# worldbench/lidarcrafter

Measured on AMD Instinct MI355X. Metric: denoising-steps/sec, nuScenes 32×1024 range image, 1/2/4/8 GPU, higher is better.
Workload: dtype f16x2-split MFMA, fp32 accumulate (fp32-class accuracy)

## Files before the change

### lidarcrafter_amd/csrc/conv_f16x2.hip

```cpp
#include "conv_f16x2_common.h"

using namespace lcconv;

namespace {

#if LC_TIMING
__device__ unsigned long long lc_dbg[32];
#endif

#ifndef LC_NP_AUX
#define LC_NP_AUX LC_DEF_AUX
#endif
template <class C, bool WIDE = false, bool EMIT = false>
__global__ __launch_bounds__(256, (C::BN > 64 && C::NTAP == 9) ? 1 : 2) void conv_f16x2_kernel(ConvArgsH a) {
    constexpr int HALO = C::HALO, NTAP = C::NTAP, BN = C::BN;
    constexpr int XR = C::XR, XW = C::XW;
    constexpr int KS = 2 * HALO + 1;
    constexpr int CB = (NTAP == 1 && WIDE) ? ((BN <= 64 && C::TH_ * C::TW_ <= 128) ? 8 : 4) : C::CB;
    constexpr int XU = CB * XR * XW, NXU = (XU + 255) / 256;
    constexpr int WU = NTAP * CB * BN, NWU = (WU + 255) / 256;
    __shared__ half8 lds[2 * XU + 2 * WU];
    __shared__ f32x4 ctab[GN_MAX_C];
    __shared__ float2 gtab[GN_MAX_G];
    half8* xh = lds;
// ... 641 lines not shown
        while (t < 4 && extent % (t * 2) == 0 && n_tiles / (t * 2) >= 256) t *= 2;
        return t;
    };
    static const int vert_env = [] { const char* e = getenv("LC_CONV_VERT"); return e ? atoi(e) : 1; }();
    static const int xcd_env = [] { const char* e = getenv("LC_CONV_XCD"); return e ? atoi(e) : 1; }();
    const int tpb_h = max_tpb(a.tiles_h), tpb_w = max_tpb(a.tiles_w);
    int vert = vert_env && tpb_h >= tpb_w;
    int tpb = vert ? tpb_h : tpb_w;
    if (C::NTAP == 1) tpb = 1;
    if (a.tpb > 0) {
        tpb = a.tpb;
        vert = vert_env && a.tiles_h % tpb == 0;
        if (!vert && a.tiles_w % tpb) tpb = 1;
    }
    if (a.part) tpb = 1;
    a.tpb = tpb;
    a.vert = vert;
    dim3 grid(a.B * a.tiles_h * a.tiles_w / tpb, ncot);
    a.xcd = (xcd_env && grid.x % 8 == 0 && grid.x >= 16) ? 1 : 0;

    if (a.xsp) {
        if constexpr (C::NTAP == 9) {
            if (a.part) grid.z = a.ksplit;
            if (a.ostats && !a.part) hipLaunchKernelGGL((conv_f16x2_ps_kernel<C, true>), grid, dim3(C::NT), 0, st, a);
            else hipLaunchKernelGGL((conv_f16x2_ps_kernel<C, false>), grid, dim3(C::NT), 0, st, a);
            return lc_launch_status();
        } else {
            return LC_EUNSUP;
        }
    }
    {
        const long long d = (const char*)a.wl - (const char*)a.wh;
        if (d <= 0 || d >= (1ll << 31)) return LC_EINVAL;
        if (d + (long long)C::NTAP * a.Cib * a.Cop * 16 >= (1ll << 31)) return LC_EUNSUP;
    }
    const int gnm = a.gn ? (a.gn_silu ? 1 : 2) : 0;
#define LC_PIPE_LAUNCH(E, G) hipLaunchKernelGGL((conv_f16x2_pipe_kernel<C, E, G>), grid, dim3(C::NT), 0, st, a)
    if (a.ostats && a.ounit == 2) {
        if constexpr (C::NTAP == 9) {
            if (gnm == 1) LC_PIPE_LAUNCH(2, 1); else if (gnm == 2) LC_PIPE_LAUNCH(2, 2); else LC_PIPE_LAUNCH(2, 0);
        } else {
            return LC_EUNSUP;
        }
    } else if (a.ostats) {
        if (gnm == 1) LC_PIPE_LAUNCH(1, 1); else if (gnm == 2) LC_PIPE_LAUNCH(1, 2); else LC_PIPE_LAUNCH(1, 0);
    } else {
// ... 333 lines not shown
extern "C" int lc_range_from_amax(const float* amax, int64_t n, float bound_mult, lc_conv_range* range, lc_stream_t s) {
    if (!amax || n <= 0 || !range || !(bound_mult >= 1.0f)) return LC_EINVAL;
    hipLaunchKernelGGL(range_from_amax_kernel, dim3(1), dim3(256), 0, lc_s(s), range, amax, (long long)n, bound_mult);
    return lc_launch_status();
}

extern "C" int lc_conv2d_ring_f16x2_fwd(const float* x, int64_t x_bs, const void* wp_hi,
                                        const void* wp_lo, const float* bias, const float* res,
                                        int64_t res_bs, float* y, int64_t y_bs, int B, int Ci,
                                        int Co, int H, int W, int ks, float out_scale, int tile_cfg,
                                        const float* gn_coeffs, int gn_cpad, int gn_silu,
                                        const lc_gn_stats_input* gn_stats, float* gn_ostats_out, int gn_ostats_unit,
                                        const float* wmeta, lc_conv_range* range, lc_stream_t s) {
    if (!x || !wp_hi || !wp_lo || !y || !wmeta || !range || B <= 0 || Ci <= 0 || Co <= 0 || H <= 0 ||
        W <= 0)
        return LC_EINVAL;
    if (ks != 1 && ks != 3) return LC_EUNSUP;
    if ((long long)H * W >= (1 << 24)) return LC_EUNSUP;
    if ((long long)Ci * H * W * 4 >= (1ll << 31) || (long long)Co * H * W * 4 >= (1ll << 31)) return LC_EUNSUP;
    ConvArgsH a;
    a.x = x; a.wh = (const half8*)wp_hi; a.wl = (const half8*)wp_lo; a.bias = bias; a.res = res;
    a.y = y; a.x_bs = x_bs; a.res_bs = res_bs; a.y_bs = y_bs;
    a.range = range; a.wmeta = wmeta;
    a.xsp = nullptr; a.xsp_bs = 0; a.xsp_c8 = 0; a.part = nullptr; a.ksplit = 0;
    a.B = B; a.Ci = Ci; a.Co = Co; a.H = H; a.W = W;
    a.Cib = (Ci + 15) / 16 * 2; a.Cop = (Co + 63) / 64 * 64;
    a.out_scale = out_scale;
    a.tiles_h = a.tiles_w = 0;
    a.gn = reinterpret_cast<const f32x4*>(gn_coeffs);
    a.Cgn = gn_cpad; a.gn_silu = gn_silu;
    a.gs = lc_gn_stats_input{nullptr, 0, 0, 0.f, nullptr, nullptr, nullptr, nullptr, 0, nullptr, nullptr};
    a.segs = STAT_SEGS_NONE;
    if (gn_stats) {
        if (gn_coeffs || gn_stats->G <= 0 || Ci % gn_stats->G) return LC_EINVAL;
        if (gn_stats->partials) {
            if (gn_stats->nch <= 0) return LC_EINVAL;
        } else {
            if (const int rc = stat_segs_from(gn_stats->os0, gn_stats->os1, Ci, Ci / gn_stats->G, LC_EINVAL, a.segs)) return rc;
            if (gn_stats->G > GN_MAX_G) return LC_EUNSUP;
        }
        a.gs = *gn_stats;
        a.gs.os0 = a.gs.os1 = nullptr;
        a.gn = reinterpret_cast<const f32x4*>(x);
        a.Cgn = gn_cpad > 0 ? gn_cpad : (Ci + 15) / 16 * 16;
    }
    a.tpb = 0;
    if (tile_cfg >= 100) { a.tpb = tile_cfg / 100; tile_cfg %= 100; }
// ... 40 lines not shown
                                           lc_conv_range* range, lc_stream_t s) {
    if (!x_split || !wp_hi || !wp_lo || (!y && !splitk_part) || !wmeta || !range || B <= 0 || Ci <= 0 ||
        Co <= 0 || H <= 0 || W <= 0)
        return LC_EINVAL;
    if (Ci % 16) return LC_EUNSUP;
    if (splitk_part && (ksplit < 2 || ksplit > Ci / 16)) return LC_EINVAL;
    if ((long long)H * W >= (1 << 24) || (long long)2 * (Ci / 8) * H * W * 16 >= (1ll << 31)) return LC_EUNSUP;
    if ((long long)Co * H * W * 4 >= (1ll << 31)) return LC_EUNSUP;
    ConvArgsH a;
    a.x = nullptr; a.wh = (const half8*)wp_hi; a.wl = (const half8*)wp_lo; a.bias = bias; a.res = res;
    a.y = y; a.x_bs = 0; a.res_bs = res_bs; a.y_bs = y_bs;
    a.range = range; a.wmeta = wmeta;
    a.B = B; a.Ci = Ci; a.Co = Co; a.H = H; a.W = W;
    a.Cib = Ci / 8; a.Cop = (Co + 63) / 64 * 64;
    if (a.wl != a.wh + (long long)9 * a.Cib * a.Cop) return LC_EINVAL;
    a.xsp = (const half8*)x_split; a.xsp_c8 = Ci / 8; a.xsp_bs = (long long)2 * (Ci / 8) * H * W;
    a.part = splitk_part; a.ksplit = splitk_part ? ksplit : 0;
    a.out_scale = out_scale;
    a.tiles_h = a.tiles_w = 0;
    a.gn = nullptr; a.Cgn = 0; a.gn_silu = 0;
    a.gs = lc_gn_stats_input{nullptr, 0, 0, 0.f, nullptr, nullptr, nullptr, nullptr, 0, nullptr, nullptr};
    a.segs = STAT_SEGS_NONE;
    a.tpb = 0;
    if (tile_cfg >= 100) { a.tpb = tile_cfg / 100; tile_cfg %= 100; }
    if (tile_cfg == 0) tile_cfg = auto_cfg_h(B, Ci < 24 ? 24 : Ci, Co, H, W, 3);
    if (pipe_stat_slots(tile_cfg, H, W) <= 0) return LC_EUNSUP;
    a.ostats = nullptr; a.oslots = 0; a.ounit = 8;
    if (gn_ostats_out && !splitk_part) {
        a.oslots = pipe_stat_slots(tile_cfg, H, W);
        if (Co % 8 || (gn_ostats_unit != 8 && gn_ostats_unit != 4)) return LC_EUNSUP;
        a.ostats = reinterpret_cast<f32x4*>(gn_ostats_out);
        a.ounit = gn_ostats_unit;
    }
    return dispatch_h<3>(tile_cfg, a, lc_s(s));
}

#include "conv_f16x2_ps1.h"

namespace {
__global__ __launch_bounds__(256) void splitk_reduce_kernel(const float* __restrict__ part, int ks,
                                                           const float* __restrict__ bias,
                                                           const float* __restrict__ res,
                                                           long long res_bs, float* __restrict__ y,
                                                           long long y_bs, int B, int Co, int HW,
                                                           float out_scale, f32x4* __restrict__ ostats,
                                                           int oslots) {
// ... 70 lines not shown
```

### lidarcrafter_amd/csrc/conv_f16x2_common.h

```cpp
#pragma once
#include <cstdlib>
#include <type_traits>

#include "common.h"
#include "f16x2.h"
#include "stats_entry.h"

#ifndef LC_EPI_MODE
#define LC_EPI_MODE 2
#endif

namespace lcconv {


__device__ __forceinline__ void epi_store(float* p, float v) {
#if LC_EPI_MODE == 2
    asm volatile("global_store_dword %0, %1, off sc1" :: "v"(p), "v"(v) : "memory");
#elif LC_EPI_MODE == 3
    asm volatile("global_store_dword %0, %1, off nt" :: "v"(p), "v"(v) : "memory");
#else
    *p = v;
#endif
}

// ... 34 lines not shown
    const float* bias;
    const float* res;
    float* y;
    lc_conv_range* range;
    const float* wmeta;
    const half8* xsp;
    long long xsp_bs;
    int xsp_c8;
    float* part;
    int ksplit;
    long long x_bs, res_bs, y_bs;
    int B, Ci, Co, H, W, Cib, Cop;
    int tiles_h, tiles_w;
    float out_scale;
    const f32x4* gn;
    int Cgn, gn_silu;
    lc_gn_stats_input gs;
    StatSegs segs;
    int tpb;
    int vert;
    int xcd;
    f32x4* ostats;
    int oslots, ounit;
};

constexpr int GN_MAX_C = 1024;

__device__ __forceinline__ f32x4 gn_row_from_stats(const lc_gn_stats_input& gs, const float* xb,
                                                   int b, int c, int C, long long HW) {
    f32x4 r = {0.f, 0.f, 0.f, 0.f};
    if (c >= C) return r;
    const int cpg = C / gs.G, g = c / cpg;
    const double* pp = gs.partials + ((long long)b * gs.G + g) * gs.nch * 2;
    double s_ = 0.0, q_ = 0.0;
    typedef double f64x2 __attribute__((ext_vector_type(2)));
    const f64x2* pv = reinterpret_cast<const f64x2*>(pp);
    for (int k0 = 0; k0 < gs.nch; k0 += 8) {
        f64x2 v[8];
#pragma unroll
        for (int k = 0; k < 8; ++k) v[k] = k0 + k < gs.nch ? pv[k0 + k] : f64x2{0.0, 0.0};
#pragma unroll
        for (int k = 0; k < 8; ++k)
            if (k0 + k < gs.nch) { s_ += v[k].x; q_ += v[k].y; }
    }
    const double n = (double)cpg * (double)HW;
    const double dm = s_ / n;
// ... 288 lines not shown
```

### lidarcrafter_amd/csrc/conv_f16x2_ps.h

```cpp
#pragma once

template <class C, bool EMIT_STATS, bool S2 = false>
__global__ __launch_bounds__(C::NT, C::NT / 256) void conv_f16x2_ps_kernel(ConvArgsH a) {
    constexpr int CB = C::CB, HALO = C::HALO, NTAP = C::NTAP, BN = C::BN;
    constexpr int XR = S2 ? 3 * C::TH_ : C::XR, XW = S2 ? 2 * C::TW_ + 1 : C::XW, XU = CB * XR * XW, WU = C::WU;
    static_assert(!S2 || (C::TH_ == 1 && NTAP == 9), "stride-2 form: 3x3, one output row per tile");
    constexpr int KS = 2 * HALO + 1;
    constexpr int NT = C::NT, NWV = NT / 64;
    constexpr int NXI = (XU + 63) / 64, NWI = (WU + 63) / 64;
    constexpr int XS = NXI * 64, WS = NWI * 64;
    constexpr int KX = (2 * NXI + NWV - 1) / NWV, KW = (2 * NWI + NWV - 1) / NWV;
    constexpr int IPW = KX + KW;
#ifndef LC_PS_SPT
#define LC_PS_SPT 0
#endif
    constexpr int SPT = LC_PS_SPT ? LC_PS_SPT : (IPW + NTAP - 1) / NTAP;
    constexpr int BUF = 2 * XS + 2 * WS + 64;
    constexpr unsigned OOB = 0x80000000u;
    __shared__ half8 lds[2 * BUF];
    const int tid = threadIdx.x;
    const int lane = tid & 63;
    const int wave = __builtin_amdgcn_readfirstlane(tid >> 6);
    const int wco = wave / C::WPX_, wpx = wave % C::WPX_;

    const int tpb = a.tpb;
    int bx = blockIdx.x;
    if (a.xcd) bx = (bx & 7) * (gridDim.x >> 3) + (bx >> 3);
    int tw_i, th_i;
    if (a.vert) {
// ... 22 lines not shown
    __amdgpu_buffer_rsrc_t rs_w = __builtin_amdgcn_make_buffer_rsrc((void*)a.wh, 0, 2u * wplane * 16u,
                                                                    0x00020000);

    unsigned voff[IPW];
    int ldsoff[IPW];
#pragma unroll
    for (int k = 0; k < IPW; ++k) {
        if (k < KX) {
            const int j = wave + k * NWV;
            const int plane = j / NXI;
            ldsoff[k] = j < 2 * NXI ? plane * XS + (j - plane * NXI) * 64 : 2 * XS + 2 * WS;
        } else {
            const int j = wave + (k - KX) * NWV;
            const int plane = j / NWI;
            ldsoff[k] = j < 2 * NWI ? 2 * XS + plane * WS + (j - plane * NWI) * 64 : 2 * XS + 2 * WS;
        }
    }
    auto set_offsets = [&](int h0t, int w0t, bool weights_too) {
#pragma unroll
        for (int k = 0; k < IPW; ++k) {
            if (k < KX) {
                const int j = wave + k * NWV;
                const int plane = j / NXI, e = (j - plane * NXI) * 64 + lane;
                const int cb = e / (XR * XW), rem = e - cb * (XR * XW);
                const int r = rem / XW, c = rem - r * XW;
                if constexpr (S2) {
                    const int ky = r;
                    int row = 2 * h0t + ky;
                    if (h0t == 0 && ky == 2) row = 2 * H + 1;
                    if (h0t == H - 1 && ky == 0) row = 2 * H + 2;
                    int col;
                    if (c <= C::TW_) { col = w0t + c; col = col >= W ? col - W : col; }
                    else col = W + w0t + (c - C::TW_ - 1);
                    const bool ok = j < 2 * NXI && e < XU && h0t < H;
                    voff[k] = ok ? (unsigned)(((plane * C8 + cb) * XROWS + row) * XCOLS + col) * 16u : OOB;
                    continue;
                }
                const int gh = h0t - HALO + r;
                int gw = w0t - HALO + c;
                gw %= W; if (gw < 0) gw += W;
                const bool ok = j < 2 * NXI && e < XU && gh >= 0 && gh < H;
                voff[k] = ok ? (unsigned)(((plane * C8 + cb) * H + gh) * W + gw) * 16u : OOB;
            } else if (weights_too) {
                const int j = wave + (k - KX) * NWV;
                const int plane = j / NWI, e = (j - plane * NWI) * 64 + lane;
                const int row = e / BN, cu = e - row * BN;
                const int tap = row / CB, cb = row - tap * CB;
                voff[k] = (j < 2 * NWI && e < WU)
                              ? ((unsigned)((tap * a.Cib + cb) * a.Cop + co0 + cu) + plane * wplane) * 16u
                              : OOB;
            }
        }
    };
    set_offsets(h0, w0, true);
    const unsigned x_chunk = (unsigned)CB * (unsigned)(XROWS * XCOLS) * 16u;
    const unsigned w_chunk = (unsigned)CB * (unsigned)a.Cop * 16u;
    auto issue_slot = [&](half8* buf, int k, unsigned xso, unsigned wso) {
        if (LC_PS_ABL & 1) return;
        if (k < KX) {
            if (!(LC_PS_ABL & 4)) lds_dma16(rs_x, (lds_vptr)(buf + ldsoff[k]), voff[k], xso);
        } else {
            if (!(LC_PS_ABL & 8)) lds_dma16(rs_w, (lds_vptr)(buf + ldsoff[k]), voff[k], wso);
        }
    };
    auto issue = [&](half8* buf, int ch) {
#pragma unroll
        for (int k = 0; k < IPW; ++k) issue_slot(buf, k, (unsigned)ch * x_chunk, (unsigned)ch * w_chunk);
    };

    f32x16 acc[C::TCO_][C::TPX_];
#pragma unroll
    for (int i = 0; i < C::TCO_; ++i)
#pragma unroll
        for (int j = 0; j < C::TPX_; ++j)
#pragma unroll
            for (int r = 0; r < 16; ++r) acc[i][j][r] = 0.0f;

    const int kh = lane >> 5, l31 = lane & 31;
    int xbase[C::TPX_];
#pragma unroll
    for (int j = 0; j < C::TPX_; ++j) {
        const int t = wpx * C::TPX_ + j;
        const int tr = t / C::TPR, tc = t - tr * C::TPR;
        xbase[j] = kh * (XR * XW) + (S2 ? 3 * tr : tr) * XW + tc * 32 + l31;
    }
    const int wbase = kh * BN + wco * C::TCO_ * 32 + l31;

    auto compute = [&](const half8* cur, half8* nxt, int nxt_ch) {
        const unsigned xso = (unsigned)nxt_ch * x_chunk, wso = (unsigned)nxt_ch * w_chunk;
        const half8* cxh = cur;
        const half8* cxl = cur + XS;
        const half8* cwh = cur + 2 * XS;
        const half8* cwl = cwh + WS;
        half8 ah[2][C::TCO_], al[2][C::TCO_], bh[2][C::TPX_], bl[2][C::TPX_];
        auto fetch = [&](int tap, int s) {
            const int dy = tap / KS, dx = tap - dy * KS;
#pragma unroll
            for (int i = 0; i < C::TCO_; ++i) {
                ah[s][i] = cwh[tap * CB * BN + wbase + i * 32];
                al[s][i] = cwl[tap * CB * BN + wbase + i * 32];
            }
#pragma unroll
            for (int j = 0; j < C::TPX_; ++j) {
                const int o = S2 ? dy * XW + (dx == 1 ? C::TW_ + 1 : (dx == 2 ? 1 : 0)) : dy * XW + dx;
                bh[s][j] = cxh[xbase[j] + o];
                bl[s][j] = cxl[xbase[j] + o];
            }
        };
        fetch(0, 0);
// ... 14 lines not shown
                        acc[i][j] = __builtin_amdgcn_mfma_f32_32x32x16_f16(al[s][i], bh[s][j], acc[i][j], 0, 0, 0);
            }
            if (LC_F16X2_TERMS & 4) {
#pragma unroll
                for (int i = 0; i < C::TCO_; ++i)
#pragma unroll
                    for (int j = 0; j < C::TPX_; ++j)
                        acc[i][j] = __builtin_amdgcn_mfma_f32_32x32x16_f16(ah[s][i], bl[s][j], acc[i][j], 0, 0, 0);
            }
#pragma unroll
            for (int i = 0; i < C::TCO_; ++i)
#pragma unroll
                for (int j = 0; j < C::TPX_; ++j)
                    acc[i][j] = __builtin_amdgcn_mfma_f32_32x32x16_f16(ah[s][i], bh[s][j], acc[i][j], 0, 0, 0);
            if (LC_PS_SCHED == 1) {
#pragma unroll
                for (int q = 0; q < 3 * C::TCO_ * C::TPX_; ++q) {
                    __builtin_amdgcn_sched_group_barrier(0x008, 1, 0);
                    __builtin_amdgcn_sched_group_barrier(0x100, 1, 0);
                }
            }
        }
        __builtin_amdgcn_sched_barrier(0);
    };

    half8* cur = lds;
    half8* nxt = lds + BUF;
    const int nchunk = a.Cib / CB;
    const int ksp = a.part ? a.ksplit : 1;
    const int ch_lo = (int)blockIdx.z * nchunk / ksp, ch_hi = ((int)blockIdx.z + 1) * nchunk / ksp;
    const int last = ch_hi - 1;
    issue(cur, ch_lo);
    const int co_wave = co0 + wco * C::TCO_ * 32 + 4 * kh;
    float bias_r[C::TCO_][16];
#pragma unroll
    for (int i = 0; i < C::TCO_; ++i)
#pragma unroll
        for (int r = 0; r < 16; ++r) {
            const int co = co_wave + i * 32 + mfma_row(r);
            bias_r[i][r] = (a.bias && co < a.Co) ? a.bias[co] : 0.0f;
        }
    float res_r[C::TCO_][C::TPX_][16];
    const float* rb = a.res ? a.res + (long long)b * a.res_bs : nullptr;
    const unsigned HW4 = (unsigned)HW * 4u;
    const __amdgpu_buffer_rsrc_t rs_yb = __builtin_amdgcn_make_buffer_rsrc(
        (void*)(a.y + (long long)b * a.y_bs), 0, (unsigned)a.Co * HW4, 0x00020000);
// ... 3 lines not shown
        const int t = wpx * C::TPX_ + j;
        const int tr = t / C::TPR, tc = t - tr * C::TPR;
        const int gh = h0 + tr, gw = w0 + tc * 32 + l31;
        return (gh < H && gw < W) ? (unsigned)(co_wave * HW + gh * W + gw) * 4u : OOB;
    };
    auto prefetch_res = [&]() {
#pragma unroll
        for (int j = 0; j < C::TPX_; ++j) {
            const unsigned vo = px_off(j);
#pragma unroll
            for (int i = 0; i < C::TCO_; ++i)
#pragma unroll
                for (int r = 0; r < 16; ++r) {
                    const int cor = i * 32 + mfma_row(r);
                    res_r[i][j][r] = (LC_PS_ABL & 16) ? 0.0f : __builtin_bit_cast(float, __builtin_amdgcn_raw_buffer_load_b32(
                        rs_rb, co_wave + cor < a.Co ? vo : OOB, (unsigned)cor * HW4, 0));
                }
        }
    };
    asm volatile("s_waitcnt vmcnt(0)" ::: "memory");
    __syncthreads();
    auto k_iter = [&](int nxt_ch) {
        if (LC_PS_ABL & 2) issue(nxt, nxt_ch);
        else compute(cur, nxt, nxt_ch);
        asm volatile("s_waitcnt vmcnt(0)" ::: "memory");
        __syncthreads();
        half8* t = cur; cur = nxt; nxt = t;
    };
    for (int tile = 0; tile < tpb; ++tile) {
        for (int ch = ch_lo; ch < last; ++ch) k_iter(ch + 1);
        if (!a.part) prefetch_res();
        const bool more = tile + 1 < tpb;
        if (more) set_offsets(h0 + dh, w0 + dw, false);
        k_iter(more ? ch_lo : last);
        if (a.part) {
            float* pb = a.part + ((long long)blockIdx.z * a.B + b) * a.Co * HW;
#pragma unroll
            for (int j = 0; j < C::TPX_; ++j) {
                const int t = wpx * C::TPX_ + j;
                const int tr = t / C::TPR, tc = t - tr * C::TPR;
                const int gh = h0 + tr, gw = w0 + tc * 32 + l31;
                const bool pok = gh < H && gw < W;
                const long long poff = (long long)gh * W + gw;
#pragma unroll
                for (int i = 0; i < C::TCO_; ++i)
#pragma unroll
                    for (int r = 0; r < 16; ++r) {
                        const int co = co_wave + i * 32 + mfma_row(r);
                        if (pok && co < a.Co) epi_store(&pb[(long long)co * HW + poff], acc[i][j][r] * out_unscale);
                        acc[i][j][r] = 0.0f;
                    }
            }
            h0 += dh; w0 += dw;
            continue;
        }
        StatAcc<PIVOT_HALF_RT> st[C::TCO_][4];
        const bool quads = a.ounit == 4, upper_quad = quads && (lane & 32);
// ... 50 lines not shown
```

### lidarcrafter_amd/csrc/conv_f16x2_s2.hip

```cpp
#include "conv_f16x2_common.h"

using namespace lcconv;

namespace {

#include "conv_f16x2_ps.h"

__global__ __launch_bounds__(256) void fir_down2_prefilter_split_kernel(
    const float* __restrict__ x, long long x_bs, half8* __restrict__ ysp, int C8, int H, int W, int nstrip, int strip_len,
    lc_conv_range* range) {
    const int Wh = W >> 1;
    const int i = blockIdx.x * 256 + threadIdx.x;
    const int c8 = blockIdx.y;
    const int b = blockIdx.z / nstrip, strip = blockIdx.z - b * nstrip;
    const float xs = range->x_scale, seen = range->amax_scaled;
    float am = 0.f;
    if (i < Wh) {
        const long long HW = (long long)H * W;
        const float* xb = x + b * x_bs + (long long)c8 * 8 * HW;
        const int R = H + 3;
        half8* yh = ysp + ((long long)b * 2 * C8 + c8) * R * W;
        half8* yl = yh + (long long)C8 * R * W;
        const int cm1 = (2 * i - 1 + W) % W, cp2 = (2 * i + 2) % W;
        constexpr float f0 = 0.125f, f1 = 0.375f, f2 = 0.375f, f3 = 0.125f;
// ... 306 lines not shown
    dim3 grid((W / 2 + 255) / 256, C / 8, B * nstrip);
    hipLaunchKernelGGL(fir_down2_prefilter_split_kernel, grid, dim3(256), 0, lc_s(s), x, (long long)x_bs,
                       reinterpret_cast<half8*>(y_split), C / 8, H, W, nstrip, strip_len, range);
    return lc_launch_status();
}

extern "C" int lc_conv2d_ring_s2_f16x2_ps_fwd(const void* x_split, const void* wp_hi, const void* wp_lo, const float* bias,
                                              float* y, int64_t y_bs, int B, int Ci, int Co, int Ho, int Wo, float out_scale,
                                              float* gn_ostats_out, int gn_ostats_unit, const float* wmeta,
                                              lc_conv_range* range, lc_stream_t s) {
    using C = S2Cfg;
    if (!x_split || !wp_hi || !wp_lo || !y || !wmeta || !range || B <= 0 || Ci <= 0 || Co <= 0 || Ho <= 0 || Wo <= 0)
        return LC_EINVAL;
    if (Ci % 16 || Ho < 2 || Wo % C::TW_) return LC_EUNSUP;
    const long long plane_units = (long long)(Ci / 8) * (2 * Ho + 3) * (2 * Wo);
    if (2 * plane_units * 16 >= (1ll << 31) || (long long)Co * Ho * Wo * 4 >= (1ll << 31)) return LC_EUNSUP;
    ConvArgsH a;
    a.x = nullptr; a.wh = (const half8*)wp_hi; a.wl = (const half8*)wp_lo; a.bias = bias; a.res = nullptr;
    a.y = y; a.x_bs = 0; a.res_bs = 0; a.y_bs = y_bs;
    a.range = range; a.wmeta = wmeta;
    a.B = B; a.Ci = Ci; a.Co = Co; a.H = Ho; a.W = Wo;
    a.Cib = Ci / 8; a.Cop = (Co + 63) / 64 * 64;
    if (a.wl != a.wh + (long long)9 * a.Cib * a.Cop) return LC_EINVAL;
    a.xsp = (const half8*)x_split; a.xsp_c8 = Ci / 8; a.xsp_bs = 2 * plane_units;
    a.part = nullptr; a.ksplit = 0;
    a.out_scale = out_scale;
    a.gn = nullptr; a.Cgn = 0; a.gn_silu = 0;
    a.gs = lc_gn_stats_input{nullptr, 0, 0, 0.f, nullptr, nullptr, nullptr, nullptr, 0, nullptr, nullptr};
    a.segs = STAT_SEGS_NONE;
    a.ostats = nullptr; a.oslots = 0; a.ounit = 8;
    if (gn_ostats_out) {
        if (Co % 8 || (gn_ostats_unit != 8 && gn_ostats_unit != 4)) return LC_EUNSUP;
        a.oslots = (int)lc_conv2d_ring_s2_stats_slots(Ho, Wo);
        a.ostats = reinterpret_cast<f32x4*>(gn_ostats_out);
        a.ounit = gn_ostats_unit;
    }
    a.tiles_h = Ho; a.tiles_w = Wo / C::TW_;
    const int ncot = (Co + C::BN - 1) / C::BN;
    const long long n_tiles = (long long)B * a.tiles_h * a.tiles_w * ncot;
    int tpb = 1;
    while (tpb < 4 && a.tiles_h % (tpb * 2) == 0 && n_tiles / (tpb * 2) >= 256) tpb *= 2;
    a.tpb = tpb; a.vert = 1;
    dim3 grid(B * a.tiles_h * a.tiles_w / tpb, ncot);
    a.xcd = (grid.x % 8 == 0 && grid.x >= 16) ? 1 : 0;
    static const int form_env = [] { const char* e = getenv("LC_S2_FORM"); return e ? atoi(e) : 2; }();
    if (form_env == 1) {
        if (a.ostats) hipLaunchKernelGGL((conv_f16x2_ps_kernel<C, true, true>), grid, dim3(C::NT), 0, lc_s(s), a);
// ... 17 lines not shown
```

### lidarcrafter_amd/ops.py

```python
from __future__ import annotations

from typing import Optional

import torch

from ._lib import check, lib

_F32 = torch.float32
_HALF = (torch.float16, torch.bfloat16)


def _stream() -> int:
    return torch.cuda.current_stream().cuda_stream


def _req(t: torch.Tensor, name: str) -> None:
    if not isinstance(t, torch.Tensor) or not t.is_cuda:
        raise RuntimeError(f"lidarcrafter_amd.ops: `{name}` must be a CUDA(HIP) tensor -- the hot "
                           "path has no CPU fallback (oracle/ holds the CPU restatement for tests)")
    if t.dtype != _F32:
        raise TypeError(f"`{name}` must be float32, got {t.dtype} (float16 / bfloat16 INPUTS are "
                        "up-cast at the op boundary, e.g. under torch.autocast; `out=` tensors and "
                        "other dtypes are not)")

# ... 815 lines not shown
            sbuf, slots = None, 0
            unit = 2 if (emit_stats is not True and int(emit_stats) in (2, 4)) else 8
            if emit_stats and PRODUCER_GN_STATS and (unit == 8 or ks == 3):
                slots = int(lib().lc_conv2d_ring_f16x2_stats_slots(B, Ci, Co, H, W, ks, int(tile_cfg)))
                if slots > 0:
                    sbuf = torch.empty((B, Co // unit, slots, 4), device=x.device, dtype=_F32)
            check(_conv_lib().lc_conv2d_ring_f16x2_fwd(x.data_ptr(), x_bs, wh.data_ptr(), wl.data_ptr(),
                                                 _p(bias), _p(res), r_bs, out.data_ptr(), y_bs, B,
                                                 Ci, Co, H, W, ks, float(out_scale),
                                                 int(tile_cfg), _p(gn_coeffs), cpad, int(gn_silu),
                                                 gs_ref, _p(sbuf), unit, packed.wmeta.data_ptr(),
                                                 packed.range_ptr(x.device), _stream()),
                  "lc_conv2d_ring_f16x2_fwd")
            if sbuf is not None:
                _attach_stats(out, _OctStatsHandle(sbuf, Co, slots, (B, H * W), unit))
        else:
            check(lib().lc_conv2d_ring_fwd(x.data_ptr(), x_bs, wp.data_ptr(), _p(bias), _p(res),
                                           r_bs, out.data_ptr(), y_bs, B, Ci, Co, H, W, ks,
                                           float(out_scale), int(tile_cfg), _stream()),
                  "lc_conv2d_ring_fwd")
    return out


def _conv2d_ring_presplit(xs: SplitAct, packed: PackedConv, weight, bias, res, out, out_scale,
                          tile_cfg, emit_stats) -> torch.Tensor:
    if xs.packed is not packed:
        raise ValueError("conv: the pre-split activation was produced for another layer "
                         "(its x_scale belongs to that layer's range record)")
    wh, wl = packed.get_f16x2(weight)
    B, Ci, H, W = xs.shape
    if Ci != packed.Ci or packed.ks not in (1, 3):
        raise ValueError("conv: pre-split input needs a 1x1 / 3x3 kernel with matching channels")
    Co = packed.Co
    dev = xs.buf.device
    if out is None:
        out = torch.empty((B, Co, H, W), device=dev, dtype=_F32)
    y_bs = _bs4(out, "out")
    if tuple(out.shape) != (B, Co, H, W):
        raise ValueError(f"conv: out shape {tuple(out.shape)} != {(B, Co, H, W)}")
    r_bs = 0
    if res is not None:
        r_bs = _bs4(res, "res")
        if tuple(res.shape) != (B, Co, H, W):
            raise ValueError("conv: residual shape mismatch")
    if bias is not None:
        _req(bias, "bias")
    _drop_stats(out)
    if packed.ks == 1:
        with _Timed("conv1x1", 2.0 * B * H * W * Co * Ci):
            check(_conv_lib().lc_conv1x1_f16x2_ps_fwd(xs.buf.data_ptr(), wh.data_ptr(), wl.data_ptr(), _p(bias), _p(res),
                                                      r_bs, out.data_ptr(), y_bs, B, Ci, Co, H, W, float(out_scale),
                                                      packed.wmeta.data_ptr(), packed.range_ptr(dev), _stream()),
                  "lc_conv1x1_f16x2_ps_fwd")
        return out
    ks = splitk_factor(B, Ci, Co, H, W) if tile_cfg == 0 else 0
    sk_cfg = 0
    if _SPLITK_FORCE and tile_cfg == 0 and Ci >= _SPLITK_FORCE[2]:
        ks, sk_cfg = _SPLITK_FORCE[0], _SPLITK_FORCE[1]
    with _Timed("conv3x3", 2.0 * B * H * W * Co * Ci * 9,
                rd=4.0 * (B * Ci * H * W + Co * Ci * 9 + (B * Co * H * W if res is not None else 0)),
                wr=4.0 * B * Co * H * W):
        sbuf, slots = None, 0
        unit = 8 if emit_stats is True else int(emit_stats or 0)
        want_stats = unit in (8, 4) and PRODUCER_GN_STATS and Co % 8 == 0
        if ks >= 2:
            part = torch.empty((ks, B, Co, H, W), device=dev, dtype=_F32)
            check(_conv_lib().lc_conv2d_ring_f16x2_ps_fwd(xs.buf.data_ptr(), wh.data_ptr(), wl.data_ptr(),
                                                    None, None, 0, None, 0, B, Ci, Co, H, W, 1.0, sk_cfg,
                                                    None, 8, part.data_ptr(), ks,
                                                    packed.wmeta.data_ptr(), packed.range_ptr(dev),
                                                    _stream()), "lc_conv2d_ring_f16x2_ps_fwd")
            if want_stats and unit == 8:
                slots = int(lib().lc_splitk_stats_slots(H, W))
                sbuf = torch.empty((B, Co // 8, slots, 4), device=dev, dtype=_F32)
            check(lib().lc_splitk_reduce(part.data_ptr(), ks, _p(bias), _p(res), r_bs, out.data_ptr(),
                                         y_bs, B, Co, H, W, float(out_scale), _p(sbuf), _stream()),
                  "lc_splitk_reduce")
        else:
            if want_stats:
                slots = int(lib().lc_conv2d_ring_f16x2_stats_slots(B, max(Ci, 24), Co, H, W, 3,
                                                                   int(tile_cfg)))
                if slots > 0:
                    sbuf = torch.empty((B, Co // unit, slots, 4), device=dev, dtype=_F32)
            check(_conv_lib().lc_conv2d_ring_f16x2_ps_fwd(xs.buf.data_ptr(), wh.data_ptr(), wl.data_ptr(),
                                                    _p(bias), _p(res), r_bs, out.data_ptr(), y_bs, B,
                                                    Ci, Co, H, W, float(out_scale), int(tile_cfg),
                                                    _p(sbuf), unit if sbuf is not None else 8, None, 0,
                                                    packed.wmeta.data_ptr(),
                                                    packed.range_ptr(dev), _stream()),
                  "lc_conv2d_ring_f16x2_ps_fwd")
        if sbuf is not None:
            _attach_stats(out, _OctStatsHandle(sbuf, Co, slots, (B, H * W), unit))
    return out


FOLD_DOWN = _os.environ.get("LC_FOLD_DOWN", "1") != "0"


def can_fold_down(Ci: int, Co: int, H: int, W: int) -> bool:
    return (FOLD_DOWN and PRESPLIT and CONV_PRECISION == "f16x2" and conv_products() == 3 and Ci % 16 == 0 and
            Co % 8 == 0 and H % 2 == 0 and H >= 4 and W % 128 == 0)


def conv_down2(x: torch.Tensor, packed: PackedConv, weight, bias, out: Optional[torch.Tensor] = None,
               emit_stats=False) -> torch.Tensor:
    x_bs = _bs4(x, "x")
    B, Ci, H, W = x.shape
    wh, wl = packed.get_f16x2(weight)
    Co = packed.Co
# ... 1553 lines not shown
```

Baseline: 285.8.

## Add 16x16x32 MFMA body for presplit 3x3 conv with three-product f16x2

Adds an alternative compute path to the presplit 3x3 convolution kernel that uses 16x16x32 MFMA instructions instead of 32x32x16. It pairs taps across the K dimension so the nine taps fit into five steps, pads the per-channel-block LDS image to a multiple of 16, and converts the 16x16 accumulators back into the 32x32 layout with permlane16 swaps before the epilogue. The path is on by default through an env flag, and a tile_cfg offset of 1000 can disable it. A microbenchmark comparing the two MFMA shapes is also added. The trade-off is slightly more MFMA slots per chunk, one zero-padded tap, and extra register pressure from the second accumulator set.

```diff
diff --git a/devtools/ubench/mfma_shape.hip b/devtools/ubench/mfma_shape.hip
--- /dev/null
+++ b/devtools/ubench/mfma_shape.hip
@@ -0,0 +1,185 @@
+#include <hip/hip_runtime.h>
+#include <stdio.h>
+#include <stdlib.h>
+#include <algorithm>
+#include <vector>
+typedef _Float16 half8 __attribute__((ext_vector_type(8)));
+typedef float f32x16 __attribute__((ext_vector_type(16)));
+typedef float f32x4 __attribute__((ext_vector_type(4)));
+
+constexpr int CBS = 400;
+constexpr int XW = 66;
+constexpr int XS = 832, WS = 1152;
+constexpr int IMG = 2 * XS + 2 * WS;
+
+__device__ __forceinline__ void fill(half8* lds, const half8* in) {
+    for (int e = threadIdx.x; e < IMG; e += blockDim.x) lds[e] = in[e];
+    __syncthreads();
+}
+
+struct Stamp { unsigned long long c0, c1, r0, r1; };
+__device__ __forceinline__ void stamp0(Stamp& s) { s.c0 = __builtin_amdgcn_s_memtime(); s.r0 = __builtin_amdgcn_s_memrealtime(); }
+__device__ __forceinline__ void stamp1(Stamp& s, unsigned long long* st) {
+    s.c1 = __builtin_amdgcn_s_memtime(); s.r1 = __builtin_amdgcn_s_memrealtime();
+    if (threadIdx.x == 0) { st[2 * blockIdx.x] = s.c1 - s.c0; st[2 * blockIdx.x + 1] = s.r1 - s.r0; }
+}
+
+__global__ __launch_bounds__(512, 2) void k32(float* out, const half8* in, unsigned long long* st, int chunks) {
+    __shared__ half8 lds[IMG];
+    fill(lds, in);
+    const int lane = threadIdx.x & 63, wave = threadIdx.x >> 6;
+    const int kh = lane >> 5, l31 = lane & 31;
+    const half8 *cxh = lds, *cxl = lds + XS, *cwh = lds + 2 * XS, *cwl = cwh + WS;
+    const int wco = wave >> 2, wpx = wave & 3;
+    const int xb = kh * CBS + wpx * XW + l31, wb = kh * 64 + wco * 32 + l31;
+    f32x16 acc[2];
+    for (int j = 0; j < 2; ++j) for (int r = 0; r < 16; ++r) acc[j][r] = 0.f;
+    Stamp s; stamp0(s);
+    for (int ch = 0; ch < chunks; ++ch) {
+        asm volatile("" ::: "memory");
+        half8 ah[2], al[2], bh[2][2], bl[2][2];
+        auto fetch = [&](int tap, int q) {
+            const int o = (tap / 3) * XW + tap % 3;
+            ah[q] = cwh[tap * 128 + wb]; al[q] = cwl[tap * 128 + wb];
+            for (int j = 0; j < 2; ++j) { bh[q][j] = cxh[xb + o + 32 * j]; bl[q][j] = cxl[xb + o + 32 * j]; }
+        };
+        fetch(0, 0);
+#pragma unroll
+        for (int tap = 0; tap < 9; ++tap) {
+            const int q = tap & 1;
+            __builtin_amdgcn_sched_barrier(0);
+            if (tap + 1 < 9) fetch(tap + 1, q ^ 1);
+            __builtin_amdgcn_sched_barrier(0);
+#pragma unroll
+            for (int j = 0; j < 2; ++j) acc[j] = __builtin_amdgcn_mfma_f32_32x32x16_f16(al[q], bh[q][j], acc[j], 0, 0, 0);
+#pragma unroll
+            for (int j = 0; j < 2; ++j) acc[j] = __builtin_amdgcn_mfma_f32_32x32x16_f16(ah[q], bl[q][j], acc[j], 0, 0, 0);
+#pragma unroll
+            for (int j = 0; j < 2; ++j) acc[j] = __builtin_amdgcn_mfma_f32_32x32x16_f16(ah[q], bh[q][j], acc[j], 0, 0, 0);
+        }
+        __builtin_amdgcn_sched_barrier(0);
+        __syncthreads();
+    }
+    stamp1(s, st);
+    float t = 0;
+    for (int j = 0; j < 2; ++j) for (int r = 0; r < 16; ++r) t += acc[j][r];
+    out[blockIdx.x * blockDim.x + threadIdx.x] = t;
+}
+
+__global__ __launch_bounds__(512, 2) void k16(float* out, const half8* in, unsigned long long* st, int chunks) {
+    __shared__ half8 lds[IMG];
+    fill(lds, in);
+    const int lane = threadIdx.x & 63, wave = threadIdx.x >> 6;
+    const int g = lane >> 4, p = lane & 15, cb = g & 1, t2 = g >> 1;
+    const int pi = (p & 3) | ((p & 4) << 1) | ((p & 8) >> 1);
+    const int wco = wave >> 2, wpx = wave & 3;
+    const int xrow = cb * CBS + wpx * XW + p, wrow = cb * 64 + wco * 32 + pi;
+    const int xb1 = xrow + t2, xb2 = xrow + t2 * XW, xb8 = xrow + t2 * XS;
+    const int wb1 = wrow + t2 * 128, wb2 = wrow + t2 * 384, wb8 = wrow + (1 - t2) * WS;
+    const half8 *cxh = lds, *cxl = lds + XS, *cwh = lds + 2 * XS, *cwl = cwh + WS;
+    f32x4 acc[2][4];
+    for (int a = 0; a < 2; ++a) for (int j = 0; j < 4; ++j) for (int r = 0; r < 4; ++r) acc[a][j][r] = 0.f;
+    Stamp s; stamp0(s);
+    for (int ch = 0; ch < chunks; ++ch) {
+        asm volatile("" ::: "memory");
+        half8 ah[2][2], al[2][2], bh[2][4], bl[2][4];
+        auto fetch = [&](int step, int q, int part) {
+            if (step < 4) {
+                const int t0 = step == 3 ? 2 : 3 * step;
+                const int o = (t0 / 3) * XW + t0 % 3, xb = step == 3 ? xb2 : xb1, wb = step == 3 ? wb2 : wb1;
+                if (part == 0) {
+                    for (int a = 0; a < 2; ++a) al[q][a] = cwl[t0 * 128 + wb + 16 * a];
+                    for (int j = 0; j < 4; ++j) bh[q][j] = cxh[xb + o + 16 * j];
+                }
+                if (part == 1) {
+                    for (int a = 0; a < 2; ++a) ah[q][a] = cwh[t0 * 128 + wb + 16 * a];
+                    for (int j = 0; j < 4; ++j) bl[q][j] = cxl[xb + o + 16 * j];
+                }
+            } else {
+                const int o = 2 * XW + 2;
+                if (part == 0) {
+                    for (int a = 0; a < 2; ++a) al[q][a] = cwh[8 * 128 + wb8 + 16 * a];
+                    for (int j = 0; j < 4; ++j) bh[q][j] = cxh[xb8 + o + 16 * j];
+                }
+                if (part == 1) for (int a = 0; a < 2; ++a) ah[q][a] = cwh[8 * 128 + wrow + 16 * a];
+            }
+        };
+        for (int part = 0; part < 2; ++part) fetch(0, 0, part);
+#pragma unroll
+        for (int step = 0; step < 5; ++step) {
+            const int q = step & 1;
+#pragma unroll
+            for (int term = 0; term < 3; ++term) {
+                if (step == 4 && term == 1) continue;
+                __builtin_amdgcn_sched_barrier(0);
+                if (step + 1 < 5) fetch(step + 1, q ^ 1, term);
+                __builtin_amdgcn_sched_barrier(0);
+                if (step == 4 && term == 2 && t2)
+                    for (int a = 0; a < 2; ++a) for (int e = 0; e < 8; ++e) ah[q][a][e] = (_Float16)0.f;
+#pragma unroll
+                for (int a = 0; a < 2; ++a)
+#pragma unroll
+                    for (int j = 0; j < 4; ++j)
+                        acc[a][j] = __builtin_amdgcn_mfma_f32_16x16x32_f16(term == 0 ? al[q][a] : ah[q][a], term == 1 ? bl[q][j] : bh[q][j], acc[a][j], 0, 0, 0);
+            }
+        }
+        __builtin_amdgcn_sched_barrier(0);
+        __syncthreads();
+    }
+    stamp1(s, st);
+    float t = 0;
+    for (int a = 0; a < 2; ++a) for (int j = 0; j < 4; ++j) for (int r = 0; r < 4; ++r) t += acc[a][j][r];
+    out[blockIdx.x * blockDim.x + threadIdx.x] = t;
+}
+
+static double median(std::vector<double> v) { std::sort(v.begin(), v.end()); return v[v.size() / 2]; }
+
+struct Arm { double cyc_per_chunk, ghz, us, tf; };
+
+template <class K>
+Arm run(K kern, const half8* in, float* out, unsigned long long* st, int chunks, int launches) {
+    const int grid = 256;
+    std::vector<unsigned long long> h(2 * grid);
+    hipEvent_t e0, e1; hipEventCreate(&e0); hipEventCreate(&e1);
+    for (int i = 0; i < launches; ++i) kern<<<grid, 512>>>(out, in, st, chunks);
+    hipEventRecord(e0);
+    for (int i = 0; i < launches; ++i) kern<<<grid, 512>>>(out, in, st, chunks);
+    hipEventRecord(e1); hipEventSynchronize(e1);
+    float ms; hipEventElapsedTime(&ms, e0, e1);
+    hipMemcpy(h.data(), st, h.size() * 8, hipMemcpyDeviceToHost);
+    std::vector<double> cyc, clk;
+    for (int b = 0; b < grid; ++b) { cyc.push_back((double)h[2 * b]); clk.push_back((double)h[2 * b] / (double)h[2 * b + 1] * 0.1); }
+    Arm a;
+    a.cyc_per_chunk = median(cyc) / chunks; a.ghz = median(clk); a.us = ms * 1e3 / launches;
+    a.tf = 2.0 * 54 * 32 * 32 * 16 * (double)chunks * 8 * grid / (a.us * 1e-6) / 1e12;
+    hipEventDestroy(e0); hipEventDestroy(e1);
+    return a;
+}
+
+int main(int argc, char** argv) {
+    const int chunks = argc > 1 ? atoi(argv[1]) : 2000, launches = argc > 2 ? atoi(argv[2]) : 100, rounds = argc > 3 ? atoi(argv[3]) : 4;
+    std::vector<_Float16> hr(IMG * 8), hz(IMG * 8, (_Float16)0.f);
+    unsigned s = 12345u;
+    for (auto& v : hr) { s = s * 1664525u + 1013904223u; v = (_Float16)(((s >> 8) & 0xFFFF) / 32768.0f - 1.0f); }
+    half8 *dr, *dz; float* out; unsigned long long* st;
+    hipMalloc(&dr, IMG * 16); hipMalloc(&dz, IMG * 16); hipMalloc(&out, 256 * 512 * 4); hipMalloc(&st, 256 * 16);
+    hipMemcpy(dr, hr.data(), IMG * 16, hipMemcpyHostToDevice);
+    hipMemcpy(dz, hz.data(), IMG * 16, hipMemcpyHostToDevice);
+    printf("# mfma_shape: %d chunks per launch, %d timed launches per arm (after %d to settle), arms alternated\n", chunks, launches, launches);
+    printf("# data   shape     cyc/chunk  in-kernel GHz  us/launch  useful TF\n");
+    std::vector<double> tf32, tf16;
+    for (int r = 0; r < rounds; ++r) {
+        const Arm a = run(k32, dr, out, st, chunks, launches), b = run(k16, dr, out, st, chunks, launches);
+        printf("random   32x32x16  %9.1f  %13.3f  %9.1f  %9.1f\n", a.cyc_per_chunk, a.ghz, a.us, a.tf);
+        printf("random   16x16x32  %9.1f  %13.3f  %9.1f  %9.1f   ratio %.4f\n", b.cyc_per_chunk, b.ghz, b.us, b.tf, b.tf / a.tf);
+        tf32.push_back(a.tf); tf16.push_back(b.tf);
+    }
+    for (int r = 0; r < 2; ++r) {
+        const Arm a = run(k32, dz, out, st, chunks, launches), b = run(k16, dz, out, st, chunks, launches);
+        printf("zero     32x32x16  %9.1f  %13.3f  %9.1f  %9.1f\n", a.cyc_per_chunk, a.ghz, a.us, a.tf);
+        printf("zero     16x16x32  %9.1f  %13.3f  %9.1f  %9.1f   ratio %.4f\n", b.cyc_per_chunk, b.ghz, b.us, b.tf, b.tf / a.tf);
+    }
+    printf("random data: median useful TF 32x32x16 %.1f, 16x16x32 %.1f, ratio %.4f (16x16x32 carries 112 MFMA slots per chunk against 108)\n",
+           median(tf32), median(tf16), median(tf16) / median(tf32));
+    return hipDeviceSynchronize() == hipSuccess ? 0 : 1;
+}
diff --git a/lidarcrafter_amd/csrc/conv_f16x2.hip b/lidarcrafter_amd/csrc/conv_f16x2.hip
--- a/lidarcrafter_amd/csrc/conv_f16x2.hip
+++ b/lidarcrafter_amd/csrc/conv_f16x2.hip
@@ -687,6 +687,13 @@
     if (a.xsp) {
         if constexpr (C::NTAP == 9) {
             if (a.part) grid.z = a.ksplit;
+            if constexpr (LC_F16X2_TERMS == 7 && !(C::NT == 512 && C::TCO_ == 2)) {
+                if (a.mfma16) {
+                    if (a.ostats && !a.part) hipLaunchKernelGGL((conv_f16x2_ps_kernel<C, true, false, true>), grid, dim3(C::NT), 0, st, a);
+                    else hipLaunchKernelGGL((conv_f16x2_ps_kernel<C, false, false, true>), grid, dim3(C::NT), 0, st, a);
+                    return lc_launch_status();
+                }
+            }
             if (a.ostats && !a.part) hipLaunchKernelGGL((conv_f16x2_ps_kernel<C, true>), grid, dim3(C::NT), 0, st, a);
             else hipLaunchKernelGGL((conv_f16x2_ps_kernel<C, false>), grid, dim3(C::NT), 0, st, a);
             return lc_launch_status();
@@ -1066,7 +1073,7 @@
     a.x = x; a.wh = (const half8*)wp_hi; a.wl = (const half8*)wp_lo; a.bias = bias; a.res = res;
     a.y = y; a.x_bs = x_bs; a.res_bs = res_bs; a.y_bs = y_bs;
     a.range = range; a.wmeta = wmeta;
-    a.xsp = nullptr; a.xsp_bs = 0; a.xsp_c8 = 0; a.part = nullptr; a.ksplit = 0;
+    a.xsp = nullptr; a.xsp_bs = 0; a.xsp_c8 = 0; a.part = nullptr; a.ksplit = 0; a.mfma16 = 0;
     a.B = B; a.Ci = Ci; a.Co = Co; a.H = H; a.W = W;
     a.Cib = (Ci + 15) / 16 * 2; a.Cop = (Co + 63) / 64 * 64;
     a.out_scale = out_scale;
@@ -1153,6 +1160,8 @@
     a.gs = lc_gn_stats_input{nullptr, 0, 0, 0.f, nullptr, nullptr, nullptr, nullptr, 0, nullptr, nullptr};
     a.segs = STAT_SEGS_NONE;
     a.tpb = 0;
+    a.mfma16 = 1;
+    if (tile_cfg >= 1000) { a.mfma16 = 0; tile_cfg -= 1000; }
     if (tile_cfg >= 100) { a.tpb = tile_cfg / 100; tile_cfg %= 100; }
     if (tile_cfg == 0) tile_cfg = auto_cfg_h(B, Ci < 24 ? 24 : Ci, Co, H, W, 3);
     if (pipe_stat_slots(tile_cfg, H, W) <= 0) return LC_EUNSUP;
diff --git a/lidarcrafter_amd/csrc/conv_f16x2_common.h b/lidarcrafter_amd/csrc/conv_f16x2_common.h
--- a/lidarcrafter_amd/csrc/conv_f16x2_common.h
+++ b/lidarcrafter_amd/csrc/conv_f16x2_common.h
@@ -80,6 +80,7 @@
     int xcd;
     f32x4* ostats;
     int oslots, ounit;
+    int mfma16;
 };
 
 constexpr int GN_MAX_C = 1024;
diff --git a/lidarcrafter_amd/csrc/conv_f16x2_ps.h b/lidarcrafter_amd/csrc/conv_f16x2_ps.h
--- a/lidarcrafter_amd/csrc/conv_f16x2_ps.h
+++ b/lidarcrafter_amd/csrc/conv_f16x2_ps.h
@@ -1,10 +1,13 @@
 #pragma once
 
-template <class C, bool EMIT_STATS, bool S2 = false>
+template <class C, bool EMIT_STATS, bool S2 = false, bool M16 = false>
 __global__ __launch_bounds__(C::NT, C::NT / 256) void conv_f16x2_ps_kernel(ConvArgsH a) {
     constexpr int CB = C::CB, HALO = C::HALO, NTAP = C::NTAP, BN = C::BN;
-    constexpr int XR = S2 ? 3 * C::TH_ : C::XR, XW = S2 ? 2 * C::TW_ + 1 : C::XW, XU = CB * XR * XW, WU = C::WU;
+    constexpr int XR = S2 ? 3 * C::TH_ : C::XR, XW = S2 ? 2 * C::TW_ + 1 : C::XW, WU = C::WU;
+    constexpr int XCB = M16 ? (XR * XW + 15) / 16 * 16 : XR * XW;
+    constexpr int XU = CB * XCB;
     static_assert(!S2 || (C::TH_ == 1 && NTAP == 9), "stride-2 form: 3x3, one output row per tile");
+    static_assert(!M16 || (!S2 && NTAP == 9 && CB == 2 && BN % 16 == 0 && LC_F16X2_TERMS == 7), "16x16x32 body: 3x3, stride 1, three products");
     constexpr int KS = 2 * HALO + 1;
     constexpr int NT = C::NT, NWV = NT / 64;
     constexpr int NXI = (XU + 63) / 64, NWI = (WU + 63) / 64;
@@ -73,7 +76,7 @@
             if (k < KX) {
                 const int j = wave + k * NWV;
                 const int plane = j / NXI, e = (j - plane * NXI) * 64 + lane;
-                const int cb = e / (XR * XW), rem = e - cb * (XR * XW);
+                const int cb = e / XCB, rem = e - cb * XCB;
                 const int r = rem / XW, c = rem - r * XW;
                 if constexpr (S2) {
                     const int ky = r;
@@ -90,7 +93,7 @@
                 const int gh = h0t - HALO + r;
                 int gw = w0t - HALO + c;
                 gw %= W; if (gw < 0) gw += W;
-                const bool ok = j < 2 * NXI && e < XU && gh >= 0 && gh < H;
+                const bool ok = j < 2 * NXI && e < XU && gh >= 0 && gh < H && (!M16 || rem < XR * XW);
                 voff[k] = ok ? (unsigned)(((plane * C8 + cb) * H + gh) * W + gw) * 16u : OOB;
             } else if (weights_too) {
                 const int j = wave + (k - KX) * NWV;
@@ -136,6 +139,27 @@
         xbase[j] = kh * (XR * XW) + (S2 ? 3 * tr : tr) * XW + tc * 32 + l31;
     }
     const int wbase = kh * BN + wco * C::TCO_ * 32 + l31;
+    const int g16 = lane >> 4, p16 = lane & 15, cb16 = g16 & 1, t16 = g16 >> 1;
+    const int pi16 = (p16 & 3) | ((p16 & 4) << 1) | ((p16 & 8) >> 1);
+    int xb1[C::TPX_], xb2[C::TPX_], xb8[C::TPX_];
+#pragma unroll
+    for (int j = 0; j < C::TPX_; ++j) {
+        const int t = wpx * C::TPX_ + j;
+        const int tr = t / C::TPR, tc = t - tr * C::TPR;
+        const int xrow = cb16 * XCB + tr * XW + tc * 32 + p16;
+        xb1[j] = xrow + t16; xb2[j] = xrow + t16 * XW; xb8[j] = xrow + t16 * XS;
+    }
+    const int wrow16 = cb16 * BN + wco * C::TCO_ * 32 + pi16;
+    const int wb1 = wrow16 + t16 * CB * BN, wb2 = wrow16 + t16 * 3 * CB * BN, wb8 = wrow16 + (1 - t16) * WS;
+    f32x4 c16[C::TCO_][C::TPX_][2][2];
+    if constexpr (M16) {
+#pragma unroll
+        for (int i = 0; i < C::TCO_; ++i)
+#pragma unroll
+            for (int j = 0; j < C::TPX_; ++j)
+#pragma unroll
+                for (int q = 0; q < 4; ++q) c16[i][j][q >> 1][q & 1] = f32x4{0.f, 0.f, 0.f, 0.f};
+    }
 
     auto compute = [&](const half8* cur, half8* nxt, int nxt_ch) {
         const unsigned xso = (unsigned)nxt_ch * x_chunk, wso = (unsigned)nxt_ch * w_chunk;
@@ -196,6 +220,119 @@
             }
         }
         __builtin_amdgcn_sched_barrier(0);
+    };
+
+    auto compute16 = [&](const half8* cur, half8* nxt, int nxt_ch) {
+        const unsigned xso = (unsigned)nxt_ch * x_chunk, wso = (unsigned)nxt_ch * w_chunk;
+        const half8* cxh = cur;
+        const half8* cxl = cur + XS;
+        const half8* cwh = cur + 2 * XS;
+        const half8* cwl = cwh + WS;
+        constexpr int TB = CB * BN;
+        constexpr int SPG = LC_PS_SPT ? LC_PS_SPT : (IPW + 13) / 14;
+        half8 ah[2][C::TCO_][2], al[2][C::TCO_][2], bh[2][C::TPX_][2], bl[2][C::TPX_][2];
+        auto fetch = [&](int step, int s, int part) {
+            if (step < 4) {
+                const int t0 = step == 3 ? 2 : 3 * step;
+                const int o = (t0 / KS) * XW + t0 % KS;
+                const int wb = step == 3 ? wb2 : wb1;
+                if (part == 0) {
+#pragma unroll
+                    for (int i = 0; i < C::TCO_; ++i)
+#pragma unroll
+                        for (int h = 0; h < 2; ++h) al[s][i][h] = cwl[t0 * TB + wb + i * 32 + h * 16];
+#pragma unroll
+                    for (int j = 0; j < C::TPX_; ++j)
+#pragma unroll
+                        for (int h = 0; h < 2; ++h) bh[s][j][h] = cxh[(step == 3 ? xb2[j] : xb1[j]) + o + h * 16];
+                }
+                if (part == 1) {
+#pragma unroll
+                    for (int i = 0; i < C::TCO_; ++i)
+#pragma unroll
+                        for (int h = 0; h < 2; ++h) ah[s][i][h] = cwh[t0 * TB + wb + i * 32 + h * 16];
+#pragma unroll
+                    for (int j = 0; j < C::TPX_; ++j)
+#pragma unroll
+                        for (int h = 0; h < 2; ++h) bl[s][j][h] = cxl[(step == 3 ? xb2[j] : xb1[j]) + o + h * 16];
+                }
+            } else {
+                const int o = 2 * XW + 2;
+                if (part == 0) {
+#pragma unroll
+                    for (int i = 0; i < C::TCO_; ++i)
+#pragma unroll
+                        for (int h = 0; h < 2; ++h) al[s][i][h] = cwh[8 * TB + wb8 + i * 32 + h * 16];
+#pragma unroll
+                    for (int j = 0; j < C::TPX_; ++j)
+#pragma unroll
+                        for (int h = 0; h < 2; ++h) bh[s][j][h] = cxh[xb8[j] + o + h * 16];
+                }
+                if (part == 1) {
+#pragma unroll
+                    for (int i = 0; i < C::TCO_; ++i)
+#pragma unroll
+                        for (int h = 0; h < 2; ++h) ah[s][i][h] = cwh[8 * TB + wrow16 + i * 32 + h * 16];
+                }
+            }
+        };
+        fetch(0, 0, 0);
+        fetch(0, 0, 1);
+#pragma unroll
+        for (int step = 0; step < 5; ++step) {
+            const int s = step & 1;
+#pragma unroll
+            for (int term = 0; term < 3; ++term) {
+                if (step == 4 && term == 1) continue;
+                const int grp = step * 3 + (step == 4 && term == 2 ? 1 : term);
+                __builtin_amdgcn_sched_barrier(0);
+                if (step + 1 < 5) fetch(step + 1, s ^ 1, term);
+#pragma unroll
+                for (int q = 0; q < SPG; ++q)
+                    if (grp * SPG + q < IPW) issue_slot(nxt, grp * SPG + q, xso, wso);
+                __builtin_amdgcn_sched_barrier(0);
+                if (step == 4 && term == 2) {
+#pragma unroll
+                    for (int i = 0; i < C::TCO_; ++i)
+#pragma unroll
+                        for (int h = 0; h < 2; ++h)
+#pragma unroll
+                            for (int e = 0; e < 8; ++e) ah[s][i][h][e] = t16 ? (_Float16)0.0f : ah[s][i][h][e];
+                }
+#pragma unroll
+                for (int i = 0; i < C::TCO_; ++i)
+#pragma unroll
+                    for (int h = 0; h < 2; ++h)
+#pragma unroll
+                        for (int j = 0; j < C::TPX_; ++j)
+#pragma unroll
+                            for (int v = 0; v < 2; ++v)
+                                c16[i][j][h][v] = __builtin_amdgcn_mfma_f32_16x16x32_f16(
+                                    term == 0 ? al[s][i][h] : ah[s][i][h], term == 1 ? bl[s][j][v] : bh[s][j][v], c16[i][j][h][v], 0, 0, 0);
+            }
+        }
+        __builtin_amdgcn_sched_barrier(0);
+    };
+    auto gather16 = [&]() {
+#if defined(__HIP_DEVICE_COMPILE__)
+#pragma unroll
+        for (int i = 0; i < C::TCO_; ++i)
+#pragma unroll
+            for (int j = 0; j < C::TPX_; ++j)
+#pragma unroll
+                for (int h = 0; h < 2; ++h) {
+#pragma unroll
+                    for (int r = 0; r < 4; ++r) {
+                        const float x = c16[i][j][h][0][r], y = c16[i][j][h][1][r];
+                        const auto sw = __builtin_amdgcn_permlane16_swap(__float_as_uint(x), __float_as_uint(y), false, false);
+                        const unsigned lo = sw[0], hi = sw[1];
+                        acc[i][j][8 * h + r] = __uint_as_float(lo);
+                        acc[i][j][8 * h + 4 + r] = __uint_as_float(hi);
+                    }
+                    c16[i][j][h][0] = f32x4{0.f, 0.f, 0.f, 0.f};
+                    c16[i][j][h][1] = f32x4{0.f, 0.f, 0.f, 0.f};
+                }
+#endif
     };
 
     half8* cur = lds;
@@ -245,6 +382,7 @@
     __syncthreads();
     auto k_iter = [&](int nxt_ch) {
         if (LC_PS_ABL & 2) issue(nxt, nxt_ch);
+        else if constexpr (M16) compute16(cur, nxt, nxt_ch);
         else compute(cur, nxt, nxt_ch);
         asm volatile("s_waitcnt vmcnt(0)" ::: "memory");
         __syncthreads();
@@ -256,6 +394,7 @@
         const bool more = tile + 1 < tpb;
         if (more) set_offsets(h0 + dh, w0 + dw, false);
         k_iter(more ? ch_lo : last);
+        if constexpr (M16) gather16();
         if (a.part) {
             float* pb = a.part + ((long long)blockIdx.z * a.B + b) * a.Co * HW;
 #pragma unroll
diff --git a/lidarcrafter_amd/csrc/conv_f16x2_s2.hip b/lidarcrafter_amd/csrc/conv_f16x2_s2.hip
--- a/lidarcrafter_amd/csrc/conv_f16x2_s2.hip
+++ b/lidarcrafter_amd/csrc/conv_f16x2_s2.hip
@@ -352,7 +352,7 @@
     a.B = B; a.Ci = Ci; a.Co = Co; a.H = Ho; a.W = Wo;
     a.Cib = Ci / 8; a.Cop = (Co + 63) / 64 * 64;
     if (a.wl != a.wh + (long long)9 * a.Cib * a.Cop) return LC_EINVAL;
-    a.xsp = (const half8*)x_split; a.xsp_c8 = Ci / 8; a.xsp_bs = 2 * plane_units;
+    a.xsp = (const half8*)x_split; a.xsp_c8 = Ci / 8; a.xsp_bs = 2 * plane_units; a.mfma16 = 0;
     a.part = nullptr; a.ksplit = 0;
     a.out_scale = out_scale;
     a.gn = nullptr; a.Cgn = 0; a.gn_silu = 0;
diff --git a/lidarcrafter_amd/ops.py b/lidarcrafter_amd/ops.py
--- a/lidarcrafter_amd/ops.py
+++ b/lidarcrafter_amd/ops.py
@@ -861,6 +861,13 @@
     return out
 
 
+PS_MFMA16 = _os.environ.get("LC_PS_MFMA16", "1") != "0"
+
+
+def _ps_cfg(tile_cfg: int) -> int:
+    return int(tile_cfg) + (0 if PS_MFMA16 else 1000)
+
+
 def _conv2d_ring_presplit(xs: SplitAct, packed: PackedConv, weight, bias, res, out, out_scale,
                           tile_cfg, emit_stats) -> torch.Tensor:
     if xs.packed is not packed:
@@ -905,7 +912,7 @@
         if ks >= 2:
             part = torch.empty((ks, B, Co, H, W), device=dev, dtype=_F32)
             check(_conv_lib().lc_conv2d_ring_f16x2_ps_fwd(xs.buf.data_ptr(), wh.data_ptr(), wl.data_ptr(),
-                                                    None, None, 0, None, 0, B, Ci, Co, H, W, 1.0, sk_cfg,
+                                                    None, None, 0, None, 0, B, Ci, Co, H, W, 1.0, _ps_cfg(sk_cfg),
                                                     None, 8, part.data_ptr(), ks,
                                                     packed.wmeta.data_ptr(), packed.range_ptr(dev),
                                                     _stream()), "lc_conv2d_ring_f16x2_ps_fwd")
@@ -923,7 +930,7 @@
                     sbuf = torch.empty((B, Co // unit, slots, 4), device=dev, dtype=_F32)
             check(_conv_lib().lc_conv2d_ring_f16x2_ps_fwd(xs.buf.data_ptr(), wh.data_ptr(), wl.data_ptr(),
                                                     _p(bias), _p(res), r_bs, out.data_ptr(), y_bs, B,
-                                                    Ci, Co, H, W, float(out_scale), int(tile_cfg),
+                                                    Ci, Co, H, W, float(out_scale), _ps_cfg(tile_cfg),
                                                     _p(sbuf), unit if sbuf is not None else 8, None, 0,
                                                     packed.wmeta.data_ptr(),
                                                     packed.range_ptr(dev), _stream()),
```

New measurement: 286.1, median of 3. No clear change (+0.1%).
